# facebookresearch/jepa

Measured on AMD Instinct MI355X. Metric: V-JEPA pretrain clips/sec (fwd+bwd+EMA), higher is better.
Workload: dtype bf16; 1 GPU; V-JEPA pretrain step ViT-L/16 16x224x224, B=24/GPU, 2 multiblock masks (vitl16.yaml); global_batch=24, per_gpu_batch=24, parallelism=dp1, hw_queues=4

## Files before the change

jepa_amd/csrc/gemm8_tn.hip:

```cpp
#include <type_traits>
#include "gemm_tile.hpp"
#include "options.hpp"

namespace {

__device__ __attribute__((aligned(256))) bf16_t g_tn_zero_row[128];

typedef __attribute__((ext_vector_type(4))) short tn_s16x4_t;
typedef __attribute__((ext_vector_type(8))) short tn_s16x8_t;

__device__ __forceinline__ bf16x8_t tn_frag(const char* p) {
  const tn_s16x4_t lo = __builtin_amdgcn_ds_read_tr16_b64_v4i16((__attribute__((address_space(3))) tn_s16x4_t*)p);
  const tn_s16x4_t hi =
      __builtin_amdgcn_ds_read_tr16_b64_v4i16((__attribute__((address_space(3))) tn_s16x4_t*)(p + 16 * 256));
  const tn_s16x8_t w = {lo[0], lo[1], lo[2], lo[3], hi[0], hi[1], hi[2], hi[3]};
  return __builtin_bit_cast(bf16x8_t, w);
}

struct TnLane {
  int row0;
  int sc8;
};

__device__ __forceinline__ void tn_issue_part(const GemmArgs& p, int q, int64_t m0, int64_t n0, int kt0, char* smem,
                                              const TnLane& tl, int wave_u) {
  const int qq = q + 1;
  const int kind = qq & 3;
  const int t = qq >> 2;
  const int64_t tok0 = (int64_t)(kt0 + t) * 64;
  char* slot = smem + ((q + 8) & 7) * LDS_PART_BYTES;
  const bool isA = (kind == 0) || (kind == 3);
  const int half = (kind == 0 || kind == 1) ? 0 : 1;
  const int64_t cbase = (isA ? m0 : n0) + half * 128;
  const int lim = (int)((isA ? p.M : p.N) - cbase - 8);
  const int rel = tl.sc8 < lim ? tl.sc8 : lim;
  const unsigned ld = (unsigned)(isA ? p.lda : p.ldb);
  const bf16_t* base = (isA ? p.A + tok0 * p.lda : p.B + tok0 * p.ldb) + cbase;
  const int64_t left = p.K - 1 - tok0;
  const int last_row = left < 63 ? (int)left : 63;
#pragma unroll
  for (int j = 0; j < 2; j++) {
    const int row = tl.row0 + 32 * j;
    const int rowc = row < last_row ? row : last_row;
    const bf16_t* src = base + (int64_t)(int)(__umul24((unsigned)rowc, ld) + rel);
    if (isA) {
      const bf16_t* zsrc = g_tn_zero_row + tl.sc8;
      src = row <= last_row ? src : zsrc;
    }
    dma16_v(src, lds_addr(slot + (j * 512 + wave_u * 64) * 16));
  }
}

struct TnFast {
  const char* base[4];
  int lim[4];
  unsigned step[2];
  unsigned row32[2];
  int tail_tile;
};
template <int KIND>
__device__ __forceinline__ void tn_issue_fast(TnFast& f, int q, char* smem, int sc8, unsigned rowoff_a, unsigned rowoff_b,
                                              int wave_u) {
  constexpr bool isA = (KIND == 0) || (KIND == 3);
  const unsigned slot = lds_addr(smem + ((q + 8) & 7) * LDS_PART_BYTES) + (unsigned)(wave_u * 64) * 16;
  const int rel = sc8 < f.lim[KIND] ? sc8 : f.lim[KIND];
  const unsigned v0 = (isA ? rowoff_a : rowoff_b) + ((unsigned)rel << 1);
  const unsigned v1 = v0 + f.row32[isA ? 0 : 1];
  dma16_sv(f.base[KIND], v0, slot);
  dma16_sv(f.base[KIND], v1, slot + 512 * 16);
  f.base[KIND] += f.step[isA ? 0 : 1];
}

#define TN_GROUP_MAX 4
struct TnGroupArgs {
  int n;
  int unit_end[TN_GROUP_MAX];
  GemmArgs g[TN_GROUP_MAX];
};
struct TnSingleArgs {
  GemmArgs g;
};

template <bool GROUPED>
__global__ __launch_bounds__(512) void gemm_tn_8phase_kernel(std::conditional_t<GROUPED, TnGroupArgs, TnSingleArgs> ga) {
  extern __shared__ __attribute__((aligned(16))) char smem[];
  const int tid = threadIdx.x, lane = tid & 63;
  const int wave_u = __builtin_amdgcn_readfirstlane(tid >> 6);
  const int wm = wave_u >> 2, wn = wave_u & 3;
  const bool late_group = wave_u >= 4;

  GemmArgs p;
  p.colpart = nullptr;
  p.lnf_rs = nullptr;
  p.lnf_c = nullptr;
  p.raster = 0;
  p.qscale = 0.f;
  p.qcols = 0;
  int logical_all;
  if constexpr (GROUPED) {
    const int l = xcd_logical(blockIdx.x, ga.unit_end[ga.n - 1]);
    int idx = 0;
#pragma unroll
    for (int i = 0; i + 1 < TN_GROUP_MAX; i++)
      if (i + 1 < ga.n && l >= ga.unit_end[i]) idx = i + 1;
    logical_all = l - (idx > 0 ? ga.unit_end[idx - 1] : 0);
    p = ga.g[idx];
  } else {
    p = ga.g;
    logical_all = xcd_logical(blockIdx.x, p.tiles_m * p.tiles_n * p.splitk);
  }
  const GemmUnit u = gemm_unit<256, 256, 64, true>(p, logical_all);
  const int64_t m0 = u.m0, n0 = u.n0;
  const int slice = u.slice, kt0 = u.kt0, nk = u.nk;
  const int last_part = 4 * nk - 2;

  f32x4_t acc[2][2][4][2];
#pragma unroll
  for (int a = 0; a < 2; a++)
#pragma unroll
    for (int b = 0; b < 2; b++)
#pragma unroll
      for (int i = 0; i < 4; i++)
#pragma unroll
        for (int j = 0; j < 2; j++) acc[a][b][i][j] = (f32x4_t){0.f, 0.f, 0.f, 0.f};
  bf16x8_t ra0[4][2], ra1[4][2], rb0[2][2], rb1[2][2];

  int a_off[4], b_off[2];
  {
    const int g = lane >> 4, jj = (lane & 15) >> 2, q4 = lane & 3;
    const int row_l = 4 * g + jj;
    const int key2 = (row_l & 7) << 1;
    const int base = row_l * 256 + (q4 & 1) * 8;
#pragma unroll
    for (int i = 0; i < 4; i++) a_off[i] = base + ((((wm * 8 + i * 2) ^ key2) | (q4 >> 1)) << 4);
#pragma unroll
    for (int j = 0; j < 2; j++) b_off[j] = base + ((((wn * 4 + j * 2) ^ key2) | (q4 >> 1)) << 4);
  }

  TnLane tl;
  tl.row0 = tid >> 4;
  tl.sc8 = ((tid & 15) ^ (((tid >> 4) & 7) << 1)) * 8;

  auto wait_landed = [&](int q) {
    wait_younger_parts<2, 3>(last_part - (q + 2));
  };
  auto mma_rd = [&](f32x4_t (&acc4)[4][2], const bf16x8_t (&rb)[2][2], const bf16x8_t (&ra)[4][2], auto nf_tag, auto&& load_frag)
                    __attribute__((always_inline)) {
    constexpr int NF = decltype(nf_tag)::value;
    __builtin_amdgcn_s_setprio(1);
#pragma unroll
    for (int ks = 0; ks < 2; ks++)
#pragma unroll
      for (int i = 0; i < 4; i++)
#pragma unroll
        for (int j = 0; j < 2; j++) {
          acc4[i][j] = __builtin_amdgcn_mfma_f32_16x16x32_bf16(rb[j][ks], ra[i][ks], acc4[i][j], 0, 0, 0);
          constexpr int dummy = 0;
          (void)dummy;
          const int m = ks * 8 + i * 2 + j;
          if constexpr (NF == 8) {
            if (m % 2 == 0) load_frag(m / 2);
          } else if constexpr (NF == 4) {
            if (m % 4 == 0) load_frag(m / 4);
          }
        }
    __builtin_amdgcn_s_setprio(0);
    if constexpr (NF == 8) {
#pragma unroll
      for (int f = 0; f < 8; f++) {
        __builtin_amdgcn_sched_group_barrier(0x008, 2, 0);
        __builtin_amdgcn_sched_group_barrier(0x100, 2, 0);
      }
    } else if constexpr (NF == 4) {
#pragma unroll
      for (int f = 0; f < 4; f++) {
        __builtin_amdgcn_sched_group_barrier(0x008, 4, 0);
        __builtin_amdgcn_sched_group_barrier(0x100, 2, 0);
      }
    }
  };
  using NF0 = std::integral_constant<int, 0>;
  using NF4 = std::integral_constant<int, 4>;
  using NF8 = std::integral_constant<int, 8>;

  TnFast fs;
  {
    const unsigned sa = (unsigned)p.lda * 128u, sb = (unsigned)p.ldb * 128u;
    fs.step[0] = sa;
    fs.step[1] = sb;
    fs.row32[0] = sa >> 1;
    fs.row32[1] = sb >> 1;
#pragma unroll
    for (int kind = 0; kind < 4; kind++) {
      const bool isA = (kind == 0) || (kind == 3);
      const int half = (kind == 0 || kind == 1) ? 0 : 1;
      const int64_t cbase = (isA ? m0 : n0) + half * 128;
      const int first = (kind == 0 || kind == 1) ? 2 : 1;
      const int64_t tok0 = (int64_t)(kt0 + first) * 64;
      fs.base[kind] = (const char*)((isA ? p.A + tok0 * p.lda : p.B + tok0 * p.ldb) + cbase);
      fs.lim[kind] = (int)((isA ? p.M : p.N) - cbase - 8);
    }
    fs.tail_tile = (p.K & 63) ? (int)((p.K + 63) / 64) - 1 - kt0 : -1;
  }
  const unsigned rowoff_a = (unsigned)tl.row0 * (unsigned)p.lda * 2u, rowoff_b = (unsigned)tl.row0 * (unsigned)p.ldb * 2u;
  auto issue_loop = [&](auto kind_tag, int q, int tile) __attribute__((always_inline)) {
    constexpr int KIND = decltype(kind_tag)::value;
    if (tile != fs.tail_tile && fs.lim[KIND] >= 0) tn_issue_fast<KIND>(fs, q, smem, tl.sc8, rowoff_a, rowoff_b, wave_u);
    else tn_issue_part(p, q, m0, n0, kt0, smem, tl, wave_u);
  };

  tn_issue_part(p, -1, m0, n0, kt0, smem, tl, wave_u);
#pragma unroll
  for (int q = 0; q < 5; q++)
    if (q <= last_part) tn_issue_part(p, q, m0, n0, kt0, smem, tl, wave_u);
  wait_landed(-1);
  section_barrier();
  if (late_group) section_barrier();
  {
    const char* slot = smem + 7 * LDS_PART_BYTES;
#pragma unroll
    for (int i = 0; i < 4; i++)
#pragma unroll
      for (int ks = 0; ks < 2; ks++) ra0[i][ks] = tn_frag(slot + a_off[i] + ks * 32 * 256);
  }
  section_barrier();
  section_barrier();

  for (int t = 0; t < nk; t++) {
#pragma unroll
    for (int ph = 0; ph < 4; ph++) {
      const int q = 4 * t + ph;
      if (ph == 0) {
        const char* slot = smem + (q & 7) * LDS_PART_BYTES;
#pragma unroll
        for (int j = 0; j < 2; j++)
#pragma unroll
          for (int ks = 0; ks < 2; ks++) rb0[j][ks] = tn_frag(slot + b_off[j] + ks * 32 * 256);
      }
      if (q + 5 <= last_part) {
        if (ph == 0) issue_loop(std::integral_constant<int, 2>{}, q + 5, t + 1);
        else if (ph == 1) issue_loop(std::integral_constant<int, 3>{}, q + 5, t + 1);
        else if (ph == 2) issue_loop(std::integral_constant<int, 0>{}, q + 5, t + 2);
        else issue_loop(std::integral_constant<int, 1>{}, q + 5, t + 2);
        wait_vmcnt<6>();
      } else {
        wait_landed(q);
      }
      section_barrier();
      const char* nslot = smem + ((q + 1) & 7) * LDS_PART_BYTES;
      if (ph == 0) {
        mma_rd(acc[0][0], rb0, ra0, NF4{}, [&](int f) { rb1[f >> 1][f & 1] = tn_frag(nslot + b_off[f >> 1] + (f & 1) * 32 * 256); });
      } else if (ph == 1) {
        mma_rd(acc[0][1], rb1, ra0, NF8{}, [&](int f) { ra1[f >> 1][f & 1] = tn_frag(nslot + a_off[f >> 1] + (f & 1) * 32 * 256); });
      } else if (ph == 2) {
        mma_rd(acc[1][1], rb1, ra1, NF8{}, [&](int f) { ra0[f >> 1][f & 1] = tn_frag(nslot + a_off[f >> 1] + (f & 1) * 32 * 256); });
      } else {
        mma_rd(acc[1][0], rb0, ra1, NF0{}, [&](int) {});
      }
      section_barrier();
    }
  }
  if (!late_group) section_barrier();

  const int elane = lane_id();
  const int efrow = elane & 15, efg = elane >> 4;
#pragma unroll
  for (int ih = 0; ih < 2; ih++)
#pragma unroll
    for (int jh = 0; jh < 2; jh++)
      gemm_epilogue<EPI_F32, 4, 2, true>(p, acc[ih][jh], m0 + ih * 128 + wm * 64, n0 + jh * 128 + wn * 32, efrow, efg,
                                         slice);
}

}

static int tn_check(const char* who, const void* dY, int64_t ldy, const void* X, int64_t ldx, const float* dW, int64_t ldw,
                    int64_t T, int64_t N1, int64_t N2) {
  VJ_CHECK_ARG(T > 0, "%s: T must be positive", who);
  VJ_CHECK_ARG(N1 % 8 == 0 && N2 % 8 == 0, "%s: N1=%ld, N2=%ld must be multiples of 8", who, (long)N1, (long)N2);
  VJ_CHECK_ARG(ldy % 8 == 0 && ldx % 8 == 0 && ldy >= N1 && ldx >= N2 && ldy < (1 << 24) && ldx < (1 << 24),
               "%s: ldy/ldx must be multiples of 8, >= N1/N2 and < 2^24", who);
  VJ_CHECK_ARG(((uintptr_t)dY % 16 == 0) && ((uintptr_t)X % 16 == 0) && ((uintptr_t)dW % 16 == 0),
               "%s: operands must be 16-byte aligned", who);
  VJ_CHECK_ARG(ldw % 4 == 0 && ldw >= N2, "%s: ldw=%ld must be a multiple of 4 and >= N2", who, (long)ldw);
  return 0;
}

static GemmArgs tn_args(const void* dY, int64_t ldy, const void* X, int64_t ldx, float* dW, int64_t ldw, int64_t T,
                        int64_t N1, int64_t N2, float alpha, float beta) {
  GemmArgs b;
  b.A = (const bf16_t*)dY; b.B = (const bf16_t*)X; b.C = dW;
  b.M = N1; b.N = N2; b.K = T; b.lda = ldy; b.ldb = ldx; b.ldc = ldw;
  b.alpha = alpha; b.beta = beta;
  b.tiles_m = (int)cdiv64(N1, 256);
  b.tiles_n = (int)cdiv64(N2, 256);
  b.ktiles_per = (int)cdiv64(T, 64);
  return b;
}

extern "C" int vj_gemm_bf16_tn_splitk(const void* dY, int64_t ldy, const void* X, int64_t ldx, float* dW, int64_t ldw,
                                      int64_t T, int64_t N1, int64_t N2, float alpha, float beta, void* ws,
                                      int64_t ws_bytes, hipStream_t stream) {
  VJ_CHECK_ARG(T >= 0 && N1 >= 0 && N2 >= 0, "vj_gemm_bf16_tn_splitk: negative dim");
  if (N1 == 0 || N2 == 0) return 0;
  if (int rc = tn_check("vj_gemm_bf16_tn_splitk", dY, ldy, X, ldx, dW, ldw, T, N1, N2)) return rc;
  VJ_CHECK_ARG(ws != nullptr && ws_bytes >= N1 * N2 * 4, "vj_gemm_bf16_tn_splitk: workspace must hold at least N1*N2 fp32");
  set_max_dynamic_lds<gemm_tn_8phase_kernel<false>>(8 * LDS_PART_BYTES);
  TnSingleArgs a;
  GemmArgs& b = a.g;
  b = tn_args(dY, ldy, X, ldx, dW, ldw, T, N1, N2, alpha, beta);
  const int nk = (int)cdiv64(T, 64);
  b.splitk = pick_splitk((int64_t)b.tiles_m * b.tiles_n, nk, 256, 1.45, 8, N1, N2, ws_bytes);
  b.ws = (float*)ws;
  vj_splitk_finish_plan(nk, b.splitk, b.ktiles_per);
  hipLaunchKernelGGL(gemm_tn_8phase_kernel<false>, dim3(b.tiles_m * b.tiles_n * b.splitk), dim3(512), 8 * LDS_PART_BYTES, stream, a);
  VJ_LAUNCH_CHECK("vj_gemm_bf16_tn_splitk");
  return vj_splitk_reduce(b, stream);
}

struct vj_tn_problem_abi {
  const void* dY; int64_t ldy;
  const void* X; int64_t ldx;
  float* dW; int64_t ldw;
  int64_t N1, N2;
};
extern "C" int vj_gemm_bf16_tn_grouped(const void* probs_v, int64_t n, int64_t T, float alpha, float beta, void* ws,
                                       int64_t ws_bytes, hipStream_t stream) {
  const vj_tn_problem_abi* pr = (const vj_tn_problem_abi*)probs_v;
  VJ_CHECK_ARG(n >= 0 && n <= TN_GROUP_MAX, "vj_gemm_bf16_tn_grouped: n=%ld (at most %d problems)", (long)n, TN_GROUP_MAX);
  VJ_CHECK_ARG(T >= 0, "vj_gemm_bf16_tn_grouped: negative T");
  TnGroupArgs a;
  a.n = 0;
  int64_t tiles = 0, out_elems = 0;
  for (int64_t i = 0; i < n; i++) {
    VJ_CHECK_ARG(pr[i].N1 >= 0 && pr[i].N2 >= 0, "vj_gemm_bf16_tn_grouped: negative dim");
    if (pr[i].N1 == 0 || pr[i].N2 == 0) continue;
    if (int rc = tn_check("vj_gemm_bf16_tn_grouped", pr[i].dY, pr[i].ldy, pr[i].X, pr[i].ldx, pr[i].dW, pr[i].ldw, T, pr[i].N1,
                          pr[i].N2))
      return rc;
    a.g[a.n] = tn_args(pr[i].dY, pr[i].ldy, pr[i].X, pr[i].ldx, pr[i].dW, pr[i].ldw, T, pr[i].N1, pr[i].N2, alpha, beta);
    tiles += (int64_t)a.g[a.n].tiles_m * a.g[a.n].tiles_n;
    out_elems += pr[i].N1 * pr[i].N2;
    a.n++;
  }
  if (a.n == 0) return 0;
  VJ_CHECK_ARG(ws != nullptr && ws_bytes >= out_elems * 4, "vj_gemm_bf16_tn_grouped: workspace must hold at least sum N1*N2 fp32");
  const int nk = (int)cdiv64(T, 64);
  int splitk = pick_splitk(tiles, nk, 256, 1.45, 8, out_elems, 1, ws_bytes);
  int ktiles_per;
  vj_splitk_finish_plan(nk, splitk, ktiles_per);
  int64_t units = 0, ws_off = 0;
  for (int i = 0; i < a.n; i++) {
    a.g[i].splitk = splitk;
    a.g[i].ktiles_per = ktiles_per;
    a.g[i].ws = (float*)((char*)ws + ws_off);
    ws_off += (int64_t)splitk * a.g[i].M * a.g[i].N * 4;
    units += (int64_t)a.g[i].tiles_m * a.g[i].tiles_n * splitk;
    a.unit_end[i] = (int)units;
  }
  for (int i = a.n; i < TN_GROUP_MAX; i++) {
    a.unit_end[i] = (int)units;
    a.g[i] = a.g[a.n - 1];
  }
  VJ_CHECK_ARG(units < (1ll << 31), "vj_gemm_bf16_tn_grouped: grid too large");
  set_max_dynamic_lds<gemm_tn_8phase_kernel<true>>(8 * LDS_PART_BYTES);
  hipLaunchKernelGGL(gemm_tn_8phase_kernel<true>, dim3((unsigned)units), dim3(512), 8 * LDS_PART_BYTES, stream, a);
  VJ_LAUNCH_CHECK("vj_gemm_bf16_tn_grouped");
  for (int i = 0; i < a.n; i++)
    if (int rc = vj_splitk_reduce(a.g[i], stream)) return rc;
  return 0;
}
```

Baseline: 334.4 clips/s.

## Specialize TN weight-grad GEMM for tiles with an out-of-range 128-half

Moves the TN 8-phase kernel body into an include-able unit and instantiates it with compile-time flags saying whether each 128-row/col half of the 256x256 tile lies inside the matrix. Tiles whose second A or B half is out of range skip the DMA issues, the MFMAs and the accumulators for that half, and use adjusted vmcnt waits. The specialized kernel is used only when some problem dimension leaves such a dead half, for example the predictor's 384 and 1152 widths. This adds four code variants and a more complex phase schedule, with some risk of wait-count or LDS-slot mistakes in the partial paths.

```diff
diff --git a/jepa_amd/csrc/gemm8_tn.hip b/jepa_amd/csrc/gemm8_tn.hip
--- a/jepa_amd/csrc/gemm8_tn.hip
+++ b/jepa_amd/csrc/gemm8_tn.hip
@@ -81,7 +81,23 @@
   GemmArgs g;
 };
 
-template <bool GROUPED>
+template <bool A1, bool B1>
+__device__ __forceinline__ constexpr bool tn_kind_live(int kind) {
+  return kind == 2 ? B1 : kind == 3 ? A1 : true;
+}
+template <bool A1, bool B1>
+__device__ __forceinline__ void tn_wait_live(int ph, int rem) {
+  int n = 0;
+#pragma unroll
+  for (int d = 1; d <= 3; d++)
+    if (d <= rem && tn_kind_live<A1, B1>((ph + 3 + d) & 3)) n++;
+  if (n >= 3) wait_vmcnt<6>();
+  else if (n == 2) wait_vmcnt<4>();
+  else if (n == 1) wait_vmcnt<2>();
+  else wait_vmcnt<0>();
+}
+
+template <bool GROUPED, bool KINDS>
 __global__ __launch_bounds__(512) void gemm_tn_8phase_kernel(std::conditional_t<GROUPED, TnGroupArgs, TnSingleArgs> ga) {
   extern __shared__ __attribute__((aligned(16))) char smem[];
   const int tid = threadIdx.x, lane = tid & 63;
@@ -110,166 +126,30 @@
     logical_all = xcd_logical(blockIdx.x, p.tiles_m * p.tiles_n * p.splitk);
   }
   const GemmUnit u = gemm_unit<256, 256, 64, true>(p, logical_all);
-  const int64_t m0 = u.m0, n0 = u.n0;
-  const int slice = u.slice, kt0 = u.kt0, nk = u.nk;
-  const int last_part = 4 * nk - 2;
-
-  f32x4_t acc[2][2][4][2];
-#pragma unroll
-  for (int a = 0; a < 2; a++)
-#pragma unroll
-    for (int b = 0; b < 2; b++)
-#pragma unroll
-      for (int i = 0; i < 4; i++)
-#pragma unroll
-        for (int j = 0; j < 2; j++) acc[a][b][i][j] = (f32x4_t){0.f, 0.f, 0.f, 0.f};
-  bf16x8_t ra0[4][2], ra1[4][2], rb0[2][2], rb1[2][2];
-
-  int a_off[4], b_off[2];
-  {
-    const int g = lane >> 4, jj = (lane & 15) >> 2, q4 = lane & 3;
-    const int row_l = 4 * g + jj;
-    const int key2 = (row_l & 7) << 1;
-    const int base = row_l * 256 + (q4 & 1) * 8;
-#pragma unroll
-    for (int i = 0; i < 4; i++) a_off[i] = base + ((((wm * 8 + i * 2) ^ key2) | (q4 >> 1)) << 4);
-#pragma unroll
-    for (int j = 0; j < 2; j++) b_off[j] = base + ((((wn * 4 + j * 2) ^ key2) | (q4 >> 1)) << 4);
-  }
-
-  TnLane tl;
-  tl.row0 = tid >> 4;
-  tl.sc8 = ((tid & 15) ^ (((tid >> 4) & 7) << 1)) * 8;
-
-  auto wait_landed = [&](int q) {
-    wait_younger_parts<2, 3>(last_part - (q + 2));
-  };
-  auto mma_rd = [&](f32x4_t (&acc4)[4][2], const bf16x8_t (&rb)[2][2], const bf16x8_t (&ra)[4][2], auto nf_tag, auto&& load_frag)
-                    __attribute__((always_inline)) {
-    constexpr int NF = decltype(nf_tag)::value;
-    __builtin_amdgcn_s_setprio(1);
-#pragma unroll
-    for (int ks = 0; ks < 2; ks++)
-#pragma unroll
-      for (int i = 0; i < 4; i++)
-#pragma unroll
-        for (int j = 0; j < 2; j++) {
-          acc4[i][j] = __builtin_amdgcn_mfma_f32_16x16x32_bf16(rb[j][ks], ra[i][ks], acc4[i][j], 0, 0, 0);
-          constexpr int dummy = 0;
-          (void)dummy;
-          const int m = ks * 8 + i * 2 + j;
-          if constexpr (NF == 8) {
-            if (m % 2 == 0) load_frag(m / 2);
-          } else if constexpr (NF == 4) {
-            if (m % 4 == 0) load_frag(m / 4);
-          }
-        }
-    __builtin_amdgcn_s_setprio(0);
-    if constexpr (NF == 8) {
-#pragma unroll
-      for (int f = 0; f < 8; f++) {
-        __builtin_amdgcn_sched_group_barrier(0x008, 2, 0);
-        __builtin_amdgcn_sched_group_barrier(0x100, 2, 0);
-      }
-    } else if constexpr (NF == 4) {
-#pragma unroll
-      for (int f = 0; f < 4; f++) {
-        __builtin_amdgcn_sched_group_barrier(0x008, 4, 0);
-        __builtin_amdgcn_sched_group_barrier(0x100, 2, 0);
-      }
+  if constexpr (!KINDS) {
+#define TN_UNIT_A1 true
+#define TN_UNIT_B1 true
+#include "gemm8_tn_unit.hpp"
+  } else {
+    const bool a1 = p.M - u.m0 > 128, b1 = p.N - u.n0 > 128;
+    if (a1 && b1) {
+#define TN_UNIT_A1 true
+#define TN_UNIT_B1 true
+#include "gemm8_tn_unit.hpp"
+    } else if (a1) {
+#define TN_UNIT_A1 true
+#define TN_UNIT_B1 false
+#include "gemm8_tn_unit.hpp"
+    } else if (b1) {
+#define TN_UNIT_A1 false
+#define TN_UNIT_B1 true
+#include "gemm8_tn_unit.hpp"
+    } else {
+#define TN_UNIT_A1 false
+#define TN_UNIT_B1 false
+#include "gemm8_tn_unit.hpp"
     }
-  };
-  using NF0 = std::integral_constant<int, 0>;
-  using NF4 = std::integral_constant<int, 4>;
-  using NF8 = std::integral_constant<int, 8>;
-
-  TnFast fs;
-  {
-    const unsigned sa = (unsigned)p.lda * 128u, sb = (unsigned)p.ldb * 128u;
-    fs.step[0] = sa;
-    fs.step[1] = sb;
-    fs.row32[0] = sa >> 1;
-    fs.row32[1] = sb >> 1;
-#pragma unroll
-    for (int kind = 0; kind < 4; kind++) {
-      const bool isA = (kind == 0) || (kind == 3);
-      const int half = (kind == 0 || kind == 1) ? 0 : 1;
-      const int64_t cbase = (isA ? m0 : n0) + half * 128;
-      const int first = (kind == 0 || kind == 1) ? 2 : 1;
-      const int64_t tok0 = (int64_t)(kt0 + first) * 64;
-      fs.base[kind] = (const char*)((isA ? p.A + tok0 * p.lda : p.B + tok0 * p.ldb) + cbase);
-      fs.lim[kind] = (int)((isA ? p.M : p.N) - cbase - 8);
-    }
-    fs.tail_tile = (p.K & 63) ? (int)((p.K + 63) / 64) - 1 - kt0 : -1;
-  }
-  const unsigned rowoff_a = (unsigned)tl.row0 * (unsigned)p.lda * 2u, rowoff_b = (unsigned)tl.row0 * (unsigned)p.ldb * 2u;
-  auto issue_loop = [&](auto kind_tag, int q, int tile) __attribute__((always_inline)) {
-    constexpr int KIND = decltype(kind_tag)::value;
-    if (tile != fs.tail_tile && fs.lim[KIND] >= 0) tn_issue_fast<KIND>(fs, q, smem, tl.sc8, rowoff_a, rowoff_b, wave_u);
-    else tn_issue_part(p, q, m0, n0, kt0, smem, tl, wave_u);
-  };
-
-  tn_issue_part(p, -1, m0, n0, kt0, smem, tl, wave_u);
-#pragma unroll
-  for (int q = 0; q < 5; q++)
-    if (q <= last_part) tn_issue_part(p, q, m0, n0, kt0, smem, tl, wave_u);
-  wait_landed(-1);
-  section_barrier();
-  if (late_group) section_barrier();
-  {
-    const char* slot = smem + 7 * LDS_PART_BYTES;
-#pragma unroll
-    for (int i = 0; i < 4; i++)
-#pragma unroll
-      for (int ks = 0; ks < 2; ks++) ra0[i][ks] = tn_frag(slot + a_off[i] + ks * 32 * 256);
-  }
-  section_barrier();
-  section_barrier();
-
-  for (int t = 0; t < nk; t++) {
-#pragma unroll
-    for (int ph = 0; ph < 4; ph++) {
-      const int q = 4 * t + ph;
-      if (ph == 0) {
-        const char* slot = smem + (q & 7) * LDS_PART_BYTES;
-#pragma unroll
-        for (int j = 0; j < 2; j++)
-#pragma unroll
-          for (int ks = 0; ks < 2; ks++) rb0[j][ks] = tn_frag(slot + b_off[j] + ks * 32 * 256);
-      }
-      if (q + 5 <= last_part) {
-        if (ph == 0) issue_loop(std::integral_constant<int, 2>{}, q + 5, t + 1);
-        else if (ph == 1) issue_loop(std::integral_constant<int, 3>{}, q + 5, t + 1);
-        else if (ph == 2) issue_loop(std::integral_constant<int, 0>{}, q + 5, t + 2);
-        else issue_loop(std::integral_constant<int, 1>{}, q + 5, t + 2);
-        wait_vmcnt<6>();
-      } else {
-        wait_landed(q);
-      }
-      section_barrier();
-      const char* nslot = smem + ((q + 1) & 7) * LDS_PART_BYTES;
-      if (ph == 0) {
-        mma_rd(acc[0][0], rb0, ra0, NF4{}, [&](int f) { rb1[f >> 1][f & 1] = tn_frag(nslot + b_off[f >> 1] + (f & 1) * 32 * 256); });
-      } else if (ph == 1) {
-        mma_rd(acc[0][1], rb1, ra0, NF8{}, [&](int f) { ra1[f >> 1][f & 1] = tn_frag(nslot + a_off[f >> 1] + (f & 1) * 32 * 256); });
-      } else if (ph == 2) {
-        mma_rd(acc[1][1], rb1, ra1, NF8{}, [&](int f) { ra0[f >> 1][f & 1] = tn_frag(nslot + a_off[f >> 1] + (f & 1) * 32 * 256); });
-      } else {
-        mma_rd(acc[1][0], rb0, ra1, NF0{}, [&](int) {});
-      }
-      section_barrier();
-    }
-  }
-  if (!late_group) section_barrier();
-
-  const int elane = lane_id();
-  const int efrow = elane & 15, efg = elane >> 4;
-#pragma unroll
-  for (int ih = 0; ih < 2; ih++)
-#pragma unroll
-    for (int jh = 0; jh < 2; jh++)
-      gemm_epilogue<EPI_F32, 4, 2, true>(p, acc[ih][jh], m0 + ih * 128 + wm * 64, n0 + jh * 128 + wn * 32, efrow, efg,
-                                         slice);
+  }
 }
 
 }
@@ -298,6 +178,9 @@
   return b;
 }
 
+static inline bool tn_has_dead_half(int64_t N1, int64_t N2) { return (N1 - 1) % 256 < 128 || (N2 - 1) % 256 < 128; }
+static inline bool tn_use_kinds(bool dead_half) { return dead_half && !(vj_opt(VJ_OPT_GEMM_DBG) & 2); }
+
 extern "C" int vj_gemm_bf16_tn_splitk(const void* dY, int64_t ldy, const void* X, int64_t ldx, float* dW, int64_t ldw,
                                       int64_t T, int64_t N1, int64_t N2, float alpha, float beta, void* ws,
                                       int64_t ws_bytes, hipStream_t stream) {
@@ -305,7 +188,7 @@
   if (N1 == 0 || N2 == 0) return 0;
   if (int rc = tn_check("vj_gemm_bf16_tn_splitk", dY, ldy, X, ldx, dW, ldw, T, N1, N2)) return rc;
   VJ_CHECK_ARG(ws != nullptr && ws_bytes >= N1 * N2 * 4, "vj_gemm_bf16_tn_splitk: workspace must hold at least N1*N2 fp32");
-  set_max_dynamic_lds<gemm_tn_8phase_kernel<false>>(8 * LDS_PART_BYTES);
+  set_max_dynamic_lds<gemm_tn_8phase_kernel<false, false>, gemm_tn_8phase_kernel<false, true>>(8 * LDS_PART_BYTES);
   TnSingleArgs a;
   GemmArgs& b = a.g;
   b = tn_args(dY, ldy, X, ldx, dW, ldw, T, N1, N2, alpha, beta);
@@ -313,7 +196,9 @@
   b.splitk = pick_splitk((int64_t)b.tiles_m * b.tiles_n, nk, 256, 1.45, 8, N1, N2, ws_bytes);
   b.ws = (float*)ws;
   vj_splitk_finish_plan(nk, b.splitk, b.ktiles_per);
-  hipLaunchKernelGGL(gemm_tn_8phase_kernel<false>, dim3(b.tiles_m * b.tiles_n * b.splitk), dim3(512), 8 * LDS_PART_BYTES, stream, a);
+  const dim3 grid(b.tiles_m * b.tiles_n * b.splitk);
+  if (tn_use_kinds(tn_has_dead_half(N1, N2))) hipLaunchKernelGGL((gemm_tn_8phase_kernel<false, true>), grid, dim3(512), 8 * LDS_PART_BYTES, stream, a);
+  else hipLaunchKernelGGL((gemm_tn_8phase_kernel<false, false>), grid, dim3(512), 8 * LDS_PART_BYTES, stream, a);
   VJ_LAUNCH_CHECK("vj_gemm_bf16_tn_splitk");
   return vj_splitk_reduce(b, stream);
 }
@@ -332,6 +217,7 @@
   TnGroupArgs a;
   a.n = 0;
   int64_t tiles = 0, out_elems = 0;
+  bool dead_half = false;
   for (int64_t i = 0; i < n; i++) {
     VJ_CHECK_ARG(pr[i].N1 >= 0 && pr[i].N2 >= 0, "vj_gemm_bf16_tn_grouped: negative dim");
     if (pr[i].N1 == 0 || pr[i].N2 == 0) continue;
@@ -341,6 +227,7 @@
     a.g[a.n] = tn_args(pr[i].dY, pr[i].ldy, pr[i].X, pr[i].ldx, pr[i].dW, pr[i].ldw, T, pr[i].N1, pr[i].N2, alpha, beta);
     tiles += (int64_t)a.g[a.n].tiles_m * a.g[a.n].tiles_n;
     out_elems += pr[i].N1 * pr[i].N2;
+    dead_half |= tn_has_dead_half(pr[i].N1, pr[i].N2);
     a.n++;
   }
   if (a.n == 0) return 0;
@@ -363,8 +250,9 @@
     a.g[i] = a.g[a.n - 1];
   }
   VJ_CHECK_ARG(units < (1ll << 31), "vj_gemm_bf16_tn_grouped: grid too large");
-  set_max_dynamic_lds<gemm_tn_8phase_kernel<true>>(8 * LDS_PART_BYTES);
-  hipLaunchKernelGGL(gemm_tn_8phase_kernel<true>, dim3((unsigned)units), dim3(512), 8 * LDS_PART_BYTES, stream, a);
+  set_max_dynamic_lds<gemm_tn_8phase_kernel<true, false>, gemm_tn_8phase_kernel<true, true>>(8 * LDS_PART_BYTES);
+  if (tn_use_kinds(dead_half)) hipLaunchKernelGGL((gemm_tn_8phase_kernel<true, true>), dim3((unsigned)units), dim3(512), 8 * LDS_PART_BYTES, stream, a);
+  else hipLaunchKernelGGL((gemm_tn_8phase_kernel<true, false>), dim3((unsigned)units), dim3(512), 8 * LDS_PART_BYTES, stream, a);
   VJ_LAUNCH_CHECK("vj_gemm_bf16_tn_grouped");
   for (int i = 0; i < a.n; i++)
     if (int rc = vj_splitk_reduce(a.g[i], stream)) return rc;
diff --git a/jepa_amd/csrc/gemm8_tn_unit.hpp b/jepa_amd/csrc/gemm8_tn_unit.hpp
--- /dev/null
+++ b/jepa_amd/csrc/gemm8_tn_unit.hpp
@@ -0,0 +1,198 @@
+{
+  constexpr bool A1 = TN_UNIT_A1, B1 = TN_UNIT_B1, FULL = A1 && B1;
+  const int64_t m0 = u.m0, n0 = u.n0;
+  const int slice = u.slice, kt0 = u.kt0, nk = u.nk;
+  const int last_part = 4 * nk - 2;
+
+  f32x4_t acc[A1 ? 2 : 1][B1 ? 2 : 1][4][2];
+#pragma unroll
+  for (int a = 0; a < (A1 ? 2 : 1); a++)
+#pragma unroll
+    for (int b = 0; b < (B1 ? 2 : 1); b++)
+#pragma unroll
+      for (int i = 0; i < 4; i++)
+#pragma unroll
+        for (int j = 0; j < 2; j++) acc[a][b][i][j] = (f32x4_t){0.f, 0.f, 0.f, 0.f};
+  bf16x8_t ra0[4][2], ra1[4][2], rb0[2][2], rb1[2][2];
+
+  int a_off[4], b_off[2];
+  {
+    const int g = lane >> 4, jj = (lane & 15) >> 2, q4 = lane & 3;
+    const int row_l = 4 * g + jj;
+    const int key2 = (row_l & 7) << 1;
+    const int base = row_l * 256 + (q4 & 1) * 8;
+#pragma unroll
+    for (int i = 0; i < 4; i++) a_off[i] = base + ((((wm * 8 + i * 2) ^ key2) | (q4 >> 1)) << 4);
+#pragma unroll
+    for (int j = 0; j < 2; j++) b_off[j] = base + ((((wn * 4 + j * 2) ^ key2) | (q4 >> 1)) << 4);
+  }
+
+  TnLane tl;
+  tl.row0 = tid >> 4;
+  tl.sc8 = ((tid & 15) ^ (((tid >> 4) & 7) << 1)) * 8;
+
+  auto wait_landed = [&](int q, int ph) {
+    if constexpr (FULL) wait_younger_parts<2, 3>(last_part - (q + 2));
+    else tn_wait_live<A1, B1>(ph, last_part - (q + 2));
+  };
+  auto mma_rd = [&](f32x4_t (&acc4)[4][2], const bf16x8_t (&rb)[2][2], const bf16x8_t (&ra)[4][2], auto nf_tag, auto&& load_frag)
+                    __attribute__((always_inline)) {
+    constexpr int NF = decltype(nf_tag)::value;
+    __builtin_amdgcn_s_setprio(1);
+#pragma unroll
+    for (int ks = 0; ks < 2; ks++)
+#pragma unroll
+      for (int i = 0; i < 4; i++)
+#pragma unroll
+        for (int j = 0; j < 2; j++) {
+          acc4[i][j] = __builtin_amdgcn_mfma_f32_16x16x32_bf16(rb[j][ks], ra[i][ks], acc4[i][j], 0, 0, 0);
+          constexpr int dummy = 0;
+          (void)dummy;
+          const int m = ks * 8 + i * 2 + j;
+          if constexpr (NF == 8) {
+            if (m % 2 == 0) load_frag(m / 2);
+          } else if constexpr (NF == 4) {
+            if (m % 4 == 0) load_frag(m / 4);
+          }
+        }
+    __builtin_amdgcn_s_setprio(0);
+    if constexpr (NF == 8) {
+#pragma unroll
+      for (int f = 0; f < 8; f++) {
+        __builtin_amdgcn_sched_group_barrier(0x008, 2, 0);
+        __builtin_amdgcn_sched_group_barrier(0x100, 2, 0);
+      }
+    } else if constexpr (NF == 4) {
+#pragma unroll
+      for (int f = 0; f < 4; f++) {
+        __builtin_amdgcn_sched_group_barrier(0x008, 4, 0);
+        __builtin_amdgcn_sched_group_barrier(0x100, 2, 0);
+      }
+    }
+  };
+  using NF0 = std::integral_constant<int, 0>;
+  using NF4 = std::integral_constant<int, 4>;
+  using NF8 = std::integral_constant<int, 8>;
+
+  TnFast fs;
+  {
+    const unsigned sa = (unsigned)p.lda * 128u, sb = (unsigned)p.ldb * 128u;
+    fs.step[0] = sa;
+    fs.step[1] = sb;
+    fs.row32[0] = sa >> 1;
+    fs.row32[1] = sb >> 1;
+#pragma unroll
+    for (int kind = 0; kind < 4; kind++) {
+      if (!tn_kind_live<A1, B1>(kind)) continue;
+      const bool isA = (kind == 0) || (kind == 3);
+      const int half = (kind == 0 || kind == 1) ? 0 : 1;
+      const int64_t cbase = (isA ? m0 : n0) + half * 128;
+      const int first = (kind == 0 || kind == 1) ? 2 : 1;
+      const int64_t tok0 = (int64_t)(kt0 + first) * 64;
+      fs.base[kind] = (const char*)((isA ? p.A + tok0 * p.lda : p.B + tok0 * p.ldb) + cbase);
+      fs.lim[kind] = (int)((isA ? p.M : p.N) - cbase - 8);
+    }
+    fs.tail_tile = (p.K & 63) ? (int)((p.K + 63) / 64) - 1 - kt0 : -1;
+  }
+  const unsigned rowoff_a = (unsigned)tl.row0 * (unsigned)p.lda * 2u, rowoff_b = (unsigned)tl.row0 * (unsigned)p.ldb * 2u;
+  auto issue_loop = [&](auto kind_tag, int q, int tile) __attribute__((always_inline)) {
+    constexpr int KIND = decltype(kind_tag)::value;
+    if (tile != fs.tail_tile && fs.lim[KIND] >= 0) tn_issue_fast<KIND>(fs, q, smem, tl.sc8, rowoff_a, rowoff_b, wave_u);
+    else tn_issue_part(p, q, m0, n0, kt0, smem, tl, wave_u);
+  };
+
+  tn_issue_part(p, -1, m0, n0, kt0, smem, tl, wave_u);
+#pragma unroll
+  for (int q = 0; q < 5; q++)
+    if (tn_kind_live<A1, B1>((q + 1) & 3) && q <= last_part) tn_issue_part(p, q, m0, n0, kt0, smem, tl, wave_u);
+  wait_landed(-1, 3);
+  section_barrier();
+  if (late_group) section_barrier();
+  {
+    const char* slot = smem + 7 * LDS_PART_BYTES;
+#pragma unroll
+    for (int i = 0; i < 4; i++)
+#pragma unroll
+      for (int ks = 0; ks < 2; ks++) ra0[i][ks] = tn_frag(slot + a_off[i] + ks * 32 * 256);
+  }
+  section_barrier();
+  section_barrier();
+
+  for (int t = 0; t < nk; t++) {
+#pragma unroll
+    for (int ph = 0; ph < 4; ph++) {
+      const int q = 4 * t + ph;
+      if (ph == 0) {
+        const char* slot = smem + (q & 7) * LDS_PART_BYTES;
+#pragma unroll
+        for (int j = 0; j < 2; j++)
+#pragma unroll
+          for (int ks = 0; ks < 2; ks++) rb0[j][ks] = tn_frag(slot + b_off[j] + ks * 32 * 256);
+      }
+      if (q + 5 <= last_part) {
+        if (ph == 0) {
+          if constexpr (B1) issue_loop(std::integral_constant<int, 2>{}, q + 5, t + 1);
+        } else if (ph == 1) {
+          if constexpr (A1) issue_loop(std::integral_constant<int, 3>{}, q + 5, t + 1);
+        } else if (ph == 2) issue_loop(std::integral_constant<int, 0>{}, q + 5, t + 2);
+        else issue_loop(std::integral_constant<int, 1>{}, q + 5, t + 2);
+        if constexpr (FULL) wait_vmcnt<6>();
+        else tn_wait_live<A1, B1>(ph, 3);
+      } else {
+        wait_landed(q, ph);
+      }
+      section_barrier();
+      const char* nslot = smem + ((q + 1) & 7) * LDS_PART_BYTES;
+      auto rd_rb1 = [&](int f) { rb1[f >> 1][f & 1] = tn_frag(nslot + b_off[f >> 1] + (f & 1) * 32 * 256); };
+      auto rd_ra1 = [&](int f) { ra1[f >> 1][f & 1] = tn_frag(nslot + a_off[f >> 1] + (f & 1) * 32 * 256); };
+      auto rd_ra0 = [&](int f) { ra0[f >> 1][f & 1] = tn_frag(nslot + a_off[f >> 1] + (f & 1) * 32 * 256); };
+      if constexpr (FULL) {
+        if (ph == 0) {
+          mma_rd(acc[0][0], rb0, ra0, NF4{}, rd_rb1);
+        } else if (ph == 1) {
+          mma_rd(acc[0][1], rb1, ra0, NF8{}, rd_ra1);
+        } else if (ph == 2) {
+          mma_rd(acc[1][1], rb1, ra1, NF8{}, rd_ra0);
+        } else {
+          mma_rd(acc[1][0], rb0, ra1, NF0{}, [&](int) {});
+        }
+      } else {
+        if (ph == 0) {
+          if constexpr (B1) mma_rd(acc[0][0], rb0, ra0, NF4{}, rd_rb1);
+          else mma_rd(acc[0][0], rb0, ra0, NF0{}, [&](int) {});
+        } else if (ph == 1) {
+          if constexpr (B1) {
+            mma_rd(acc[0][1], rb1, ra0, NF0{}, [&](int) {});
+          } else if constexpr (A1) {
+#pragma unroll
+            for (int f = 0; f < 8; f++) rd_ra1(f);
+          }
+        } else if (ph == 2) {
+          if constexpr (!A1) {
+#pragma unroll
+            for (int f = 0; f < 8; f++) rd_ra0(f);
+          }
+        } else {
+          if constexpr (A1) {
+            const char* qslot = smem + (q & 7) * LDS_PART_BYTES;
+            mma_rd(acc[1][0], rb0, ra1, NF8{},
+                   [&](int f) { ra0[f >> 1][f & 1] = tn_frag(qslot + a_off[f >> 1] + (f & 1) * 32 * 256); });
+          }
+        }
+      }
+      section_barrier();
+    }
+  }
+  if (!late_group) section_barrier();
+
+  const int elane = lane_id();
+  const int efrow = elane & 15, efg = elane >> 4;
+#pragma unroll
+  for (int ih = 0; ih < (A1 ? 2 : 1); ih++)
+#pragma unroll
+    for (int jh = 0; jh < (B1 ? 2 : 1); jh++)
+      gemm_epilogue<EPI_F32, 4, 2, true>(p, acc[ih][jh], m0 + ih * 128 + wm * 64, n0 + jh * 128 + wn * 32, efrow, efg,
+                                         slice);
+}
+#undef TN_UNIT_A1
+#undef TN_UNIT_B1
```

Measured after the change: 335.7 clips/s, median of 6. About the same (+0.4%).
